# GlobalArrays/ga

Measured on AMD Instinct MI355X. Metric: GiB/s device-resident 2-D strided f64 accumulate, 64 MiB patch; % HBM peak, higher is better.
Workload: dtype f64; 1 GPU; H; patch=2-D f64 2048x4096 patch, ld 8192 (64 MiB payload), payload_bytes=67108864, parallelism=owner-aligned x1 (no collective)

## Files before the change

### ga_amd/_lib.py

```python
import ctypes
import os

_HERE = os.path.dirname(os.path.abspath(__file__))
LIB_PATH = os.path.join(_HERE, "libga_amd.so")
GA_LIB_PATH = os.path.join(_HERE, "libga_amd_ga.so")
DIAG_LIB_PATH = os.path.join(_HERE, "libga_amd_diag.so")

c_int_p = ctypes.POINTER(ctypes.c_int)
c_ll_p = ctypes.POINTER(ctypes.c_longlong)


class DoubleComplex(ctypes.Structure):
    _fields_ = [("real", ctypes.c_double), ("imag", ctypes.c_double)]


class SingleComplex(ctypes.Structure):
    _fields_ = [("real", ctypes.c_float), ("imag", ctypes.c_float)]


c_void_pp = ctypes.POINTER(ctypes.c_void_p)

SIGNATURES = {
    "comex_init": (ctypes.c_int, []),
    "comex_init_args": (ctypes.c_int, [c_int_p, ctypes.c_void_p]),
# ... 333 lines not shown
    "gaamd_iov_path_counts": (ctypes.c_int, [ctypes.POINTER(ctypes.c_ulonglong)]),
    "gaamd_host_parallel": (ctypes.c_int, [ctypes.c_int, ctypes.CFUNCTYPE(None, ctypes.c_int, ctypes.c_void_p),
                                           ctypes.c_void_p]),
    "gaamd_one_pass_count": (ctypes.c_ulonglong, []),
    "gaamd_segment_cache_reuse": (ctypes.c_ulonglong, []),
    "gaamd_segment_remaps": (ctypes.c_ulonglong, []),
    "gaamd_segment_cache_trims": (ctypes.c_ulonglong, []),
    "gaamd_segment_kind": (ctypes.c_int, [ctypes.c_void_p]),
    "gaamd_vmm_access_retries": (ctypes.c_ulonglong, []),
    "gaamd_vmm_exchange_selftest": (ctypes.c_int, [ctypes.c_int]),
    "gaamd_owner_counts": (ctypes.c_int, [ctypes.POINTER(ctypes.c_ulonglong)]),
    "gaamd_peers_unmapped": (ctypes.c_int, []),
    "gaamd_plan_strided": (ctypes.c_int, [ctypes.c_int, ctypes.c_void_p, c_int_p, ctypes.c_void_p, c_int_p, c_int_p,
                                          ctypes.c_int, ctypes.c_ulonglong, ctypes.c_ulonglong,
                                          ctypes.POINTER(ctypes.c_longlong)]),
    "gaamd_set_tuning": (ctypes.c_int, [ctypes.c_char_p, ctypes.c_int]),
    "gaamd_get_tuning": (ctypes.c_int, [ctypes.c_char_p]),
    "gaamd_device_count": (ctypes.c_int, []),
    "gaamd_set_device": (ctypes.c_int, [ctypes.c_int]),
    "gaamd_stream": (ctypes.c_void_p, []),
    "gaamd_stream_at": (ctypes.c_void_p, [ctypes.c_int]),
    "gaamd_dev_malloc": (ctypes.c_void_p, [ctypes.c_size_t]),
    "gaamd_dev_free": (ctypes.c_int, [ctypes.c_void_p]),
    "gaamd_host_malloc": (ctypes.c_void_p, [ctypes.c_size_t]),
    "gaamd_host_free": (ctypes.c_int, [ctypes.c_void_p]),
    "gaamd_memcpy": (ctypes.c_int, [ctypes.c_void_p, ctypes.c_void_p, ctypes.c_size_t]),
    "gaamd_memcpy2d": (ctypes.c_int, [ctypes.c_void_p, ctypes.c_size_t, ctypes.c_void_p, ctypes.c_size_t,
                                      ctypes.c_size_t, ctypes.c_size_t]),
    "gaamd_memset": (ctypes.c_int, [ctypes.c_void_p, ctypes.c_int, ctypes.c_size_t]),
    "gaamd_sync": (ctypes.c_int, [ctypes.c_void_p]),
# ... 178 lines not shown
```

### ga_amd/csrc/comex.cpp

```cpp
#include "comex_impl.hpp"
#include "../../include/ga_amd.h"
#include <hip/hip_version.h>
#include <stdio.h>
#include <stdlib.h>
#include <string.h>
#include <time.h>
#include <unistd.h>
#include <sched.h>
#include <deque>
#include <memory>
#include <algorithm>

#ifndef GAAMD_ROCM_PATH
#define GAAMD_ROCM_PATH "/opt/rocm"
#endif

namespace gaamd {

static std::vector<std::vector<int>> g_groups;

std::vector<int> group_members(int group) {
    Runtime &r = rt();
    std::vector<int> m;
    if (group == COMEX_GROUP_WORLD) {
// ... 345 lines not shown
            dv.dev = remote_view(world, dst, dlo, dhi);
            dv.hbm = segment_kind_of(world, (const char *)dst + dlo) == 1;
        } else {
            sv.dev = remote_view(world, src, slo, shi);
            sv.hbm = segment_kind_of(world, (const char *)src + slo) == 1;
            dv = local_view(dst, dlo, dhi, true, true);
        }
    } else {
        local_views(src, slo, shi, dst, dlo, dhi, sv, dv, hdl != nullptr);
    }
    if (dv.bounce) view_rows(dv, ds, count, levels, kind == X_ACC ? rb : count[0]);
    const bool bounce_only = (needs_sync(sv) || needs_sync(dv)) && !sv.staged && !dv.staged;
    const bool host_side = (needs_sync(sv) || needs_sync(dv)) && !bounce_only;
    const bool peer = kind == X_GET && world != r.rank && r.peer_src(world);
    if (peer) g_peer_gets.fetch_add(1, std::memory_order_relaxed);
    int si = 0;
    hipStream_t st;
    {
        std::lock_guard<std::mutex> g(r.launch_mu);
        stamp(1);
        if (host_side) sched_join_write(span_of(dv.dev, dlo, dhi));
        else si = sched_pick(span_of(sv.dev, slo, shi), span_of(dv.dev, dlo, dhi), payload_bytes(rb, count, levels));
        st = r.streams[si];
        stamp(2);
        int rc = launch_strided(cop, scale, sv.dev, ss, dv.dev, ds, count, levels, st, last_launch_info(), 0, ~0ull,
                                false, peer);
        stamp(3);
        if (rc == kErrPeerOrdered) rc = get_via_scratch(sv.dev, ss, dv.dev, ds, count, levels, st);
        if (rc) fatal("strided %s launch failed (code %d): misaligned elements or bad descriptor",
                      kind == X_ACC ? "acc" : (kind == X_PUT ? "put" : "get"), rc);
        if (host_side) sched_sync_all();
    }
    const bool synced = host_side || bounce_only || (!hdl && r.blocking_sync);
    if (!host_side && synced) {
        if (dv.hbm) sched_wait_flag(si);
        else GA_HIP(hipStreamSynchronize(st));
    }
    if (world != r.rank && !synced && !r.direct_pending.empty()) r.direct_pending[world] = 1;
    if (r.debug)
        fprintf(stderr, "[ga_amd %d] %s -> %d levels %d count0 %d rows %d: src %s dst %s stream %d\n", r.rank,
                kind == X_ACC ? "acc" : (kind == X_PUT ? "put" : "get"), world, levels, count[0],
// ... 620 lines not shown
        return 0;
    }
    if (!strcmp(key, "vmm_window")) {
        if (!out || nout < 2) return -1;
        vmm_window_usage(&out[0], &out[1]);
        return 0;
    }
    if (!strcmp(key, "pinned_threads")) {
        if (out && nout >= 1) out[0] = views_pinned_threads();
        return 0;
    }
    if (!strcmp(key, "iov_host_sides")) {
        if (out && nout >= 1) out[0] = g_iov_host_sides.load(std::memory_order_relaxed);
        return 0;
    }
    return -1;
}

int gaamd_iov_path_counts(unsigned long long counts[4]) {
    for (int k = 0; k < 4; ++k) counts[k] = g_iov_path[k].load(std::memory_order_relaxed);
    return 0;
}

int gaamd_toggle_counts(unsigned long long counts[3]) {
    for (int k = 0; k < 3; ++k) counts[k] = g_toggle[k].load(std::memory_order_relaxed);
    return 0;
}

int gaamd_route_counts(unsigned long long counts[4]) {
    for (int k = 0; k < 4; ++k) counts[k] = g_route[k].load(std::memory_order_relaxed);
// ... 9 lines not shown
```

### ga_amd/csrc/gaamd_kernels.h

```cpp
#pragma once
#include <stdint.h>
#include <hip/hip_runtime.h>
#include "../../include/comex.h"

namespace gaamd {

constexpr int kMaxLevels = 7;
constexpr int kOpCopy = 0;

struct FastDiv {
    uint32_t d, m, s;
    __host__ __device__ inline uint32_t div(uint32_t n) const {
#if defined(__HIP_DEVICE_COMPILE__)
        uint32_t hi = __umulhi(n, m);
#else
        uint32_t hi = (uint32_t)(((uint64_t)n * m) >> 32);
#endif
        return (uint32_t)(((uint64_t)hi + n) >> s);
    }
};
FastDiv make_fastdiv(uint32_t d);

struct alignas(16) Scale16 { uint64_t w[2]; };

// ... 30 lines not shown
Tuning &tuning();

struct LaunchInfo {
    int kind;
    int width;
    int unroll;
    int launches;
    uint64_t blocks;
    int block;
    int levels;
    int aligned;
    int sys;
};

constexpr int kErrPeerOrdered = -10;
int launch_strided(int op, const void *scale, const void *src, const int *src_stride,
                   void *dst, const int *dst_stride, const int *count, int stride_levels,
                   hipStream_t stream, LaunchInfo *info,
                   uint64_t row_begin = 0, uint64_t row_end = ~0ull, bool plan_only = false,
                   bool src_peer = false);

void side_span_host(const int *stride, const int *count, int stride_levels, int64_t row_bytes,
                    int64_t *lo, int64_t *hi);

int elem_size(int op);

constexpr int kPatchMaxLevels = 6;
constexpr int kPatchErrNdim = -2;
constexpr int kPatchErrCount = -3;
constexpr int kPatchErrOp = -4;
constexpr int kPatchErrScalar = -5;
constexpr int kPatchErrStride = -6;
constexpr int kPatchErrRange = -7;
constexpr int kPatchErrAlign = -8;
constexpr int kPatchErrOverlap = -11;
// ... 159 lines not shown
```

### ga_amd/csrc/gaamd_kernels.hip

```cpp
#pragma clang fp contract(off)

#include "gaamd_kernels.h"
#include "gaamd_device.hpp"
#include <string.h>
#include <algorithm>
#include <type_traits>
#include <atomic>
#include <vector>
#include <utility>
#include <mutex>
#include <cmath>

namespace gaamd {

FastDiv make_fastdiv(uint32_t d) {
    FastDiv f;
    f.d = d ? d : 1;
    uint32_t l = 0;
    while ((1ull << l) < f.d) ++l;
    f.s = l;
    f.m = (uint32_t)((((1ull << 32) * ((1ull << l) - f.d)) / f.d) + 1);
    return f;
}

// ... 105 lines not shown
        const int64_t c0 = (int64_t)chunk * (BS * U) - shift;
        const bool full = c0 >= 0 && c0 + BS * U <= (int64_t)d.nvec;
        chunk_op<OP, W, U, BS, SYS>(sp, dp, c0 + threadIdx.x, d.nvec, full, op);
    }
}

struct Desc2D {
    const char *src;
    char *dst;
    int64_t s_str, d_str;
    FastDiv chunk_div;
    uint32_t row0;
};

template <class OP, int W, int BS, bool SYS = false>
__global__ __launch_bounds__(BS) void k_rows2d(const Desc2D d, const OP op) {
    const uint32_t w = blockIdx.x;
    const uint32_t rl = d.chunk_div.div(w);
    const uint32_t chunk = w - rl * d.chunk_div.d;
    const int64_t r = (int64_t)(d.row0 + rl);
    const int64_t v = (int64_t)chunk * BS + threadIdx.x;
    const char *sp = d.src + r * d.s_str + v * W;
    char *dp = d.dst + r * d.d_str + v * W;
    typename Vec<W>::T a, b;
    if constexpr (SYS) {
        if constexpr (OP::kReadsDst) b = vload<W, true>(dp);
        a = vload_sys<W>(sp);
        if constexpr (!OP::kReadsDst) b = a;
    } else {
        a = vload<W, true>(sp);
        b = a;
        if constexpr (OP::kReadsDst) b = vload<W, true>(dp);
    }
    vstore<W, kNtStore>(dp, op.template apply<W>(b, a));
}

template <int LV>
struct DescND {
    const char *src;
    char *dst;
    int64_t s_str[LV], d_str[LV];
    FastDiv cnt[LV];
    FastDiv chunk_div;
    uint32_t row0;
};

template <class OP, int W, int BS, int LV>
__global__ __launch_bounds__(BS) void k_rowsnd(const DescND<LV> d, const OP op) {
    const uint32_t w = blockIdx.x;
// ... 366 lines not shown
static int flat_block_threads(int W) { return W == 16 ? 64 : 256; }
static uint64_t flat_block_items(int W) { return W == 16 ? 64 : 256ull * 4; }

template <int W> struct DefaultU { static constexpr int value = W == 16 ? 1 : (W == 8 ? 2 : (W == 4 ? 4 : 8)); };
static int unroll_for(int W) {
    switch (W) {
    case 16: return DefaultU<16>::value;
    case 8: return DefaultU<8>::value;
    case 4: return DefaultU<4>::value;
    case 2: return DefaultU<2>::value;
    default: return DefaultU<1>::value;
    }
}
constexpr int kSysBS = 256;

template <class OP, int W, int BS, bool SYS = false>
static hipError_t go_rows2(const Desc &d, const OP &op, uint64_t blocks, hipStream_t st) {
    constexpr int U = DefaultU<W>::value;
    Desc2 e;
    e.src = d.src;
    e.dst = d.dst;
    e.s_str = d.levels ? d.s_str[0] : 0;
    e.d_str = d.levels ? d.d_str[0] : 0;
    e.row0 = d.row0;
    e.nvec = d.nvec;
    e.chunks = d.chunks;
    e.items = (uint32_t)d.items;
    e.chunk_div = d.chunk_div;
    e.align_mask = d.align_mask;
    if constexpr (U == 1) {
        if (!d.align_mask && blocks == e.items && d.nvec % (uint32_t)BS == 0) {
            Desc2D f;
            f.src = d.src;
            f.dst = d.dst;
            f.s_str = e.s_str;
            f.d_str = e.d_str;
            f.chunk_div = d.chunk_div;
            f.row0 = d.row0;
            hipLaunchKernelGGL((k_rows2d<OP, W, BS, SYS>), dim3((uint32_t)blocks), dim3(BS), 0, st, f, op);
            return hipGetLastError();
        }
    }
    hipLaunchKernelGGL((k_rows2<OP, W, U, BS, SYS>), dim3((uint32_t)blocks), dim3(BS), 0, st, e, op);
    return hipGetLastError();
}

// ... 117 lines not shown
}

static hipError_t dispatch(int op, const void *scale, const Plan &p, const Desc &d, uint64_t blocks, hipStream_t st) {
    switch (op) {
    case kOpCopy: return dispatch_op(p, d, CopyOp{}, blocks, st);
    case COMEX_ACC_INT: { AccInt o; int32_t s; memcpy(&s, scale, 4); o.s = (uint32_t)s; return dispatch_op(p, d, o, blocks, st); }
    case COMEX_ACC_LNG: { AccLng o; int64_t s; memcpy(&s, scale, 8); o.s = (uint64_t)s; return dispatch_op(p, d, o, blocks, st); }
    case COMEX_ACC_FLT: { AccFlt o; memcpy(&o.s, scale, 4); return dispatch_op(p, d, o, blocks, st); }
    case COMEX_ACC_DBL: { AccDbl o; memcpy(&o.s, scale, 8); return dispatch_op(p, d, o, blocks, st); }
    case COMEX_ACC_CPL: { AccCpl o; float s[2]; memcpy(s, scale, 8); o.sr = s[0]; o.si = s[1]; return dispatch_op(p, d, o, blocks, st); }
    case COMEX_ACC_DCP: { AccDcp o; double s[2]; memcpy(s, scale, 16); o.sr = s[0]; o.si = s[1]; return dispatch_op(p, d, o, blocks, st); }
    }
    return hipErrorInvalidValue;
}


static bool rows_may_overlap(const int64_t *str, const uint32_t *cnt, int L, int64_t row_bytes) {
    int64_t s[kMaxLevels];
    uint32_t c[kMaxLevels];
    int n = 0;
    for (int j = 0; j < L; ++j)
        if (cnt[j] > 1) { s[n] = str[j] < 0 ? -str[j] : str[j]; c[n] = cnt[j]; ++n; }
    for (int i = 1; i < n; ++i)
        for (int k = i; k > 0 && s[k] < s[k - 1]; --k) { std::swap(s[k], s[k - 1]); std::swap(c[k], c[k - 1]); }
    int64_t extent = row_bytes;
    for (int i = 0; i < n; ++i) {
        if (s[i] < extent) return true;
        extent = s[i] * (int64_t)(c[i] - 1) + extent;
    }
    return false;
// ... 167 lines not shown

void side_span_host(const int *stride, const int *count, int stride_levels, int64_t row_bytes,
                    int64_t *lo, int64_t *hi) {
    int64_t str[kMaxLevels];
    uint32_t cnt[kMaxLevels];
    for (int j = 0; j < stride_levels && j < kMaxLevels; ++j) {
        str[j] = stride[j];
        cnt[j] = count[j + 1] < 0 ? 0 : (uint32_t)count[j + 1];
    }
    side_span(str, cnt, stride_levels, row_bytes, *lo, *hi);
}

int launch_strided(int op, const void *scale, const void *src, const int *src_stride,
                   void *dst, const int *dst_stride, const int *count, int stride_levels,
                   hipStream_t stream, LaunchInfo *info, uint64_t row_begin, uint64_t row_end, bool plan_only,
                   bool src_peer) {
    const Tuning &tn = g_tuning;
    if (info) memset(info, 0, sizeof(*info));
    if (stride_levels < 0 || stride_levels > kMaxLevels) return -2;
    if (!count || count[0] <= 0) return -3;
    const int esz = elem_size(op);
    if (!esz) return -4;
    if (op != kOpCopy && !scale) return -5;
    if (stride_levels > 0 && (!src_stride || !dst_stride)) return -6;

    int64_t row_bytes = (op == kOpCopy) ? count[0] : (int64_t)(count[0] / esz) * esz;
    uint64_t rows = 1;
    for (int j = 1; j <= stride_levels; ++j) {
        if (count[j] < 0) return -3;
        rows *= (uint64_t)count[j];
    }
// ... 119 lines not shown
        for (int j = 0; j < L; ++j) any = any || (ds[j] & (int64_t)d.align_mask) != 0;
        if (!any) d.align_mask = 0;
    }
    d.chunks = (d.nvec + per_chunk - 1 + (d.align_mask ? per_chunk - 1 : 0)) / per_chunk;
    d.chunk_div = make_fastdiv(d.chunks);

    const uint64_t lim = (1ull << 31) - 1;
    uint64_t rows_per_launch = rows;
    if (kind == KK_ROWS) rows_per_launch = std::min<uint64_t>(rows, lim / d.chunks);
    if (kind == KK_FLAT) rows_per_launch = std::min<uint64_t>(rows, lim / d.nvec);
    if (kind == KK_SERIAL || kind == KK_ORDERED) rows_per_launch = rows;
    if (rows_per_launch == 0) return -9;

    int launches = 0;
    uint64_t total_blocks = 0;
    for (uint64_t r0 = row_begin; r0 < row_end; r0 += rows_per_launch) {
        const uint64_t nr = std::min<uint64_t>(rows_per_launch, row_end - r0);
        d.row0 = (uint32_t)r0;
        d.rows = (uint32_t)nr;
        uint64_t blocks = 1;
        if (kind == KK_ROWS) {
            d.items = nr * d.chunks;
            blocks = d.items;
            if (src_peer && L > 1 && blocks > 65536) blocks = 65536;
        } else if (kind == KK_FLAT) {
            d.items = nr * d.nvec;
            const uint64_t per = flat_block_items(W);
            blocks = (d.items + per - 1) / per;
        } else {
            d.items = nr;
            if (p.variant == 4) {
                const uint32_t gx = (d.nvec + 255u) / 256u;
                blocks = (uint64_t)gx * cols_sum_slices(gx, (uint32_t)nr);
            }
            else if (p.variant == 3)
                blocks = (uint64_t)((d.nvec + 255u) / 256u) * ((nr + kColsAtomicRows - 1) / kColsAtomicRows);
            else if (p.cw) blocks = (d.nvec + (uint32_t)p.cw - 1) / (uint32_t)p.cw;
            else if (p.variant) blocks = (d.nvec + 63u) / 64u;
        }
        if (blocks > lim) blocks = lim;
        if (!plan_only) {
            hipError_t e = dispatch(op, scale, p, d, blocks, stream);
            if (e != hipSuccess) return -100 - (int)e;
        }
        ++launches;
        total_blocks += blocks;
    }
    if (!plan_only) g_kind_count[kind] += (unsigned long long)launches;
    if (info) {
        info->kind = kind;
        info->width = W;
        info->unroll = (kind == KK_ROWS) ? U : (kind == KK_ORDERED ? p.variant : 0);
        info->launches = launches;
        info->blocks = total_blocks;
        info->block = (kind == KK_ROWS) ? BS
                      : (kind == KK_FLAT ? flat_block_threads(W)
                                         : ((kind == KK_ORDERED && !p.variant) ? kOrderedBS
                                            : (p.variant == 4 || p.variant == 3 ? 256 : (p.cw ? KC_NW * 64 : 64))));
        info->levels = L;
        info->aligned = d.align_mask ? 1 : 0;
        info->sys = src_peer ? 1 : 0;
    }
    return 0;
}

}
```

### ga_amd/csrc/plumbing.hip

```cpp
#include "gaamd_kernels.h"
#include "runtime.hpp"
#include <string.h>
#include <stdlib.h>
#include <dlfcn.h>

namespace gaamd {

LaunchInfo g_last;
LaunchInfo *last_launch_info() { return &g_last; }

static hipStream_t stream_of(void *s) {
    if (s) return (hipStream_t)s;
    Runtime &r = rt();
    if (r.stream) return r.stream;
    return nullptr;
}

__device__ __forceinline__ uint64_t splitmix64_at(uint64_t seed, uint64_t i) {
    uint64_t z = seed + (i + 1) * 0x9E3779B97F4A7C15ULL;
    z = (z ^ (z >> 30)) * 0xBF58476D1CE4E5B9ULL;
    z = (z ^ (z >> 27)) * 0x94D049BB133111EBULL;
    return z ^ (z >> 31);
}

__global__ __launch_bounds__(256) void k_fill(void *dst, long n, int type, uint64_t seed) {
    for (long i = (long)blockIdx.x * blockDim.x + threadIdx.x; i < n; i += (long)gridDim.x * blockDim.x) {
// ... 302 lines not shown
    if (!strcmp(key, "flat_line_min")) return &t.flat_line_min;
    if (!strcmp(key, "ordered_cols")) return &t.ordered_cols;
    if (!strcmp(key, "iov_lds")) return &t.iov_lds;
    return nullptr;
}

int gaamd_set_tuning(const char *key, int value) {
    if (!strcmp(key, "streams")) {
        Runtime &r = rt();
        if (!r.initialized || value < 1 || value > 8) return -1;
        std::lock_guard<std::mutex> g(r.launch_mu);
        const int old = (int)r.streams.size();
        sched_resize(value);
        return old;
    }
    int *f = tuning_field(key);
    if (!f) return -1;
    if (!strcmp(key, "block") && value != 0 && value != 64 && value != 128) return -1;
    const int old = *f;
    *f = value;
    return old;
}

int gaamd_get_tuning(const char *key) {
    if (!strcmp(key, "streams")) return (int)rt().streams.size();
    int *f = tuning_field(key);
    return f ? *f : -1;
}

int gaamd_device_count(void) {
    int n = 0;
    if (hipGetDeviceCount(&n) != hipSuccess) {
        (void)hipGetLastError();
        return 0;
    }
    return n;
}

int gaamd_set_device(int dev) { return hipSetDevice(dev) == hipSuccess ? 0 : -1; }
void *gaamd_stream(void) { return rt().stream; }
// ... 16 lines not shown
    hipDeviceptr_t base = nullptr;
    size_t size = 0;
    if (hipMemGetAddressRange(&base, &size, (hipDeviceptr_t)p) == hipSuccess) addr_event('f', p, size, -1);
    else (void)hipGetLastError();
    return hipFree(p) == hipSuccess ? 0 : -1;
}

void *gaamd_host_malloc(size_t bytes) {
    void *p = nullptr;
    if (hipHostMalloc(&p, bytes, hipHostMallocMapped | hipHostMallocPortable) != hipSuccess) return nullptr;
    return p;
}
int gaamd_host_free(void *p) { return hipHostFree(p) == hipSuccess ? 0 : -1; }

int gaamd_memcpy(void *dst, const void *src, size_t bytes) {
    return hipMemcpy(dst, src, bytes, hipMemcpyDefault) == hipSuccess ? 0 : -1;
}
int gaamd_memcpy2d(void *dst, size_t dpitch, const void *src, size_t spitch, size_t width, size_t height) {
    return hipMemcpy2D(dst, dpitch, src, spitch, width, height, hipMemcpyDefault) == hipSuccess ? 0 : -1;
}
int gaamd_memset(void *dst, int value, size_t bytes) {
    return hipMemset(dst, value, bytes) == hipSuccess ? 0 : -1;
}
int gaamd_sync(void *stream) {
    Runtime &r = rt();
    if (!stream && r.initialized) {
        std::lock_guard<std::mutex> g(r.launch_mu);
        sched_sync_all();
        return 0;
    }
    hipStream_t s = stream_of(stream);
    hipError_t e = s ? hipStreamSynchronize(s) : hipDeviceSynchronize();
    return e == hipSuccess ? 0 : -(int)e;
}

int gaamd_join(void) {
// ... 63 lines not shown
```

### ga_amd/csrc/runtime.hpp

```cpp
#pragma once
#include <stdint.h>
#include <stddef.h>
#include <atomic>
#include <vector>
#include <mutex>
#include <thread>
#include <hip/hip_runtime_api.h>
#include "../../include/ga_amd.h"

namespace gaamd {

[[noreturn]] void fatal(const char *fmt, ...);
void trace(int level, const char *fmt, ...) __attribute__((format(printf, 2, 3)));

#define GA_HIP(call)                                                                  \
    do {                                                                              \
        hipError_t e_ = (call);                                                       \
        if (e_ != hipSuccess)                                                         \
            ::gaamd::fatal("%s failed: %s (%s:%d)", #call, hipGetErrorString(e_),     \
                           __FILE__, __LINE__);                                       \
    } while (0)

#define GA_ASSERT(cond, msg)                                                          \
    do {                                                                              \
// ... 145 lines not shown

Runtime &rt();

void boot_init();
void boot_allgather(const void *send, void *recv, size_t bytes);
void boot_barrier();
void boot_finalize();

void segment_cache_flush();
void sched_init(int nstreams, int pull_streams = 0);
void sched_fini();
void sched_resize(int nstreams);
void own_write_guard(const Span &dst);
int sched_pick(const Span &src, const Span &dst, uint64_t payload = 0, int prefer = -1);
void sched_join();
void sched_wait_flag(int s);
void sched_flag_init();
void sched_flag_fini();
void sched_join_write(const Span &dst);
void sched_sync_all();
void sched_publish_all();
extern std::atomic<bool> g_publish_conservative;
uint64_t sched_track(int s);
bool sched_complete(int s, uint64_t seq, bool wait);
uint64_t sched_epoch();

void wire_init();
void wire_finalize();
void wire_detach();
bool wire_active();
// ... 29 lines not shown
```

### ga_amd/csrc/sched.cpp

```cpp
#include <atomic>
#include "runtime.hpp"
#include "gaamd_kernels.h"
#include <string.h>
#include <stdlib.h>
#include <deque>
#include <algorithm>

namespace gaamd {

namespace {
constexpr int kHist = 64;
struct Entry {
    int stream;
    Span src, dst;
};
std::vector<Entry> g_hist;
std::vector<hipEvent_t> g_ev;
int g_rr = 0;
int g_base = -1;
unsigned g_base_waited = 0;

inline bool overlap(const Span &a, const Span &b) { return a.lo < b.hi && b.lo < a.hi && a.lo < a.hi && b.lo < b.hi; }

constexpr uint64_t kMarkEvery = 16;
struct Mark {
    uint64_t seq;
    hipEvent_t ev;
};
struct Marks {
    uint64_t issued = 0, done = 0, marked = 0;
    std::deque<Mark> q;
};
std::vector<Marks> g_marks;
std::vector<hipEvent_t> g_mark_pool;
std::mutex g_marks_mu;

void marks_reset_done() {
    for (Marks &m : g_marks) {
        m.done = m.marked = m.issued;
        for (const Mark &k : m.q) g_mark_pool.push_back(k.ev);
        m.q.clear();
    }
}

void mark_now(int s) {
    Marks &m = g_marks[s];
    if (m.marked == m.issued) return;
    hipEvent_t e;
    if (g_mark_pool.empty()) GA_HIP(hipEventCreateWithFlags(&e, hipEventDisableTiming));
    else { e = g_mark_pool.back(); g_mark_pool.pop_back(); }
    GA_HIP(hipEventRecord(e, rt().streams[s]));
    m.q.push_back({m.issued, e});
    m.marked = m.issued;
}
}

uint64_t sched_track(int s) {
    std::lock_guard<std::mutex> g(g_marks_mu);
    if (s < 0 || s >= (int)g_marks.size()) return 0;
    Marks &m = g_marks[s];
    const uint64_t seq = ++m.issued;
    if (seq - m.marked >= kMarkEvery) mark_now(s);
    return seq;
}

bool sched_complete(int s, uint64_t seq, bool wait) {
    std::unique_lock<std::mutex> g(g_marks_mu);
    if (seq == 0 || s < 0 || s >= (int)g_marks.size()) return true;
    Marks &m = g_marks[s];
    if (seq <= m.done) return true;
    if (m.marked < seq) mark_now(s);
    while (!m.q.empty()) {
        const Mark k = m.q.front();
        hipError_t e = hipEventQuery(k.ev);
        if (e == hipErrorNotReady && wait) {
            g.unlock();
            e = hipEventSynchronize(k.ev);
            g.lock();
            if (m.q.empty() || m.q.front().ev != k.ev) {
                if (m.done >= seq) return true;
                continue;
// ... 22 lines not shown
    r.user_streams = n;
    n += pull;
    r.streams.assign(1, r.stream);
    for (int i = 1; i < n; ++i) {
        hipStream_t s;
        GA_HIP(hipStreamCreateWithFlags(&s, hipStreamDefault));
        r.streams.push_back(s);
    }
    g_ev.assign(n, nullptr);
    for (int i = 0; i < n; ++i) GA_HIP(hipEventCreateWithFlags(&g_ev[i], hipEventDisableTiming));
    std::lock_guard<std::mutex> g(g_marks_mu);
    g_marks.assign(n, Marks());
    g_hist.clear();
    g_rr = 0;
    g_base = -1;
    sched_flag_init();
}

void sched_resize(int n) {
    Runtime &r = rt();
    const int pull = (int)r.streams.size() - r.user_streams;
    sched_sync_all();
    sched_fini();
    r.streams.clear();
    sched_init(n, pull);
}

static std::vector<hipEvent_t> g_pub_ev;
std::atomic<bool> g_publish_conservative{false};

void sched_fini() {
    Runtime &r = rt();
    for (hipEvent_t e : g_pub_ev) (void)hipEventDestroy(e);
    g_pub_ev.clear();
    for (size_t i = 1; i < r.streams.size(); ++i) (void)hipStreamDestroy(r.streams[i]);
    for (hipEvent_t e : g_ev) (void)hipEventDestroy(e);
    g_ev.clear();
    std::lock_guard<std::mutex> g(g_marks_mu);
    marks_reset_done();
    for (hipEvent_t e : g_mark_pool) (void)hipEventDestroy(e);
    g_mark_pool.clear();
    g_marks.clear();
    r.streams.clear();
    g_hist.clear();
}

static void wait_on(int waiter, int producer) {
    Runtime &r = rt();
    GA_HIP(hipEventRecord(g_ev[producer], r.streams[producer]));
    GA_HIP(hipStreamWaitEvent(r.streams[waiter], g_ev[producer], 0));
}

void sched_join() {
    Runtime &r = rt();
    const int n = (int)r.streams.size();
    if (n > 1) {
        for (int x = 1; x < n; ++x) wait_on(0, x);
        for (int x = 1; x < n; ++x) wait_on(x, 0);
    }
    g_hist.clear();
    g_base = -1;
}

void sched_join_write(const Span &dst) {
    own_write_guard(dst);
    sched_join();
}

void sched_sync_all() {
    Runtime &r = rt();
    for (hipStream_t s : r.streams) GA_HIP(hipStreamSynchronize(s));
    for (uint8_t &p : r.direct_pending) p = 0;
    {
        std::lock_guard<std::mutex> g(g_marks_mu);
        marks_reset_done();
    }
    g_hist.clear();
    g_base = -1;
}

void sched_publish_all() {
    Runtime &r = rt();
    while (g_pub_ev.size() < r.streams.size()) {
        hipEvent_t e;
        GA_HIP(hipEventCreateWithFlags(&e, hipEventDisableTiming | hipEventReleaseToSystem));
        g_pub_ev.push_back(e);
    }
    for (size_t i = 0; i < r.streams.size(); ++i) GA_HIP(hipEventRecord(g_pub_ev[i], r.streams[i]));
    sched_sync_all();
}

namespace {
uint64_t *g_flag_host = nullptr, *g_flag_dev = nullptr;
std::vector<uint64_t> g_flag_seq;
}

void sched_flag_init() {
// ... 1 lines not shown
    GA_HIP(hipHostMalloc((void **)&g_flag_host, 64 * sizeof(uint64_t), hipHostMallocMapped | hipHostMallocCoherent));
    GA_HIP(hipHostGetDevicePointer((void **)&g_flag_dev, g_flag_host, 0));
    memset(g_flag_host, 0, 64 * sizeof(uint64_t));
    g_flag_seq.assign(64, 0);
    const int rc = launch_flag(g_flag_dev + 63, 0, rt().stream);
    if (rc) fatal("completion flag launch failed (%d)", rc);
    GA_HIP(hipStreamSynchronize(rt().stream));
}

void sched_wait_flag(int s) {
    Runtime &r = rt();
    uint64_t v;
    volatile uint64_t *f;
    {
        std::lock_guard<std::mutex> g(r.launch_mu);
        sched_flag_init();
        if (s < 0 || s >= 64) fatal("stream index %d out of range", s);
        v = ++g_flag_seq[s];
        const int rc = launch_flag(g_flag_dev + s, v, r.streams[s]);
        if (rc) fatal("completion flag launch failed (%d)", rc);
        f = g_flag_host + s;
    }
    for (unsigned long spins = 0; __atomic_load_n(f, __ATOMIC_ACQUIRE) < v; ++spins) {
        if ((spins & 0xfffff) == 0xfffff) {
            const hipError_t e = hipStreamQuery(r.streams[s]);
            if (e == hipSuccess) break;
            if (e != hipErrorNotReady) fatal("stream failed: %s", hipGetErrorString(e));
        }
        __builtin_ia32_pause();
    }
}

void sched_flag_fini() {
    if (g_flag_host) (void)hipHostFree(g_flag_host);
    g_flag_host = g_flag_dev = nullptr;
    g_flag_seq.clear();
}

constexpr uint64_t kBigPayload = 192ull << 20;
constexpr uint64_t kSmallPayload = 8ull << 20;

int sched_pick(const Span &src, const Span &dst, uint64_t payload, int prefer) {
    Runtime &r = rt();
    own_write_guard(dst);
    const int n = (int)r.streams.size();
    if (n <= 1) return 0;
    const int nu = std::max(1, std::min(r.user_streams, n));
    if ((int)g_hist.size() >= kHist) {
        const int s0 = g_hist.front().stream;
        bool one = g_base < 0 || g_base == s0;
        for (const Entry &e : g_hist) one = one && e.stream == s0;
        if (one) {
            g_hist.clear();
            if (g_base != s0) g_base_waited = 1u << s0;
            g_base = s0;
        } else {
            sched_join();
        }
// ... 16 lines not shown
        }
    } else {
        s = last;
        for (int x = 0; x < n; ++x)
            if (x != s && (mask & (1u << x))) wait_on(s, x);
    }
    if (g_base >= 0 && !(g_base_waited & (1u << s))) {
        wait_on(s, g_base);
        g_base_waited |= 1u << s;
        if (g_base_waited == (1u << n) - 1) g_base = -1;
    }
    g_hist.push_back({s, src, dst});
    return s;
}

}
```

### include/ga_amd.h

```cpp
#ifndef GA_AMD_H
#define GA_AMD_H

#include <stddef.h>

#if defined(__cplusplus)
extern "C" {
#endif

#define GAAMD_OP_COPY 0

typedef int (*gaamd_allgather_fn)(const void *send, void *recv, size_t bytes, void *ctx);
typedef int (*gaamd_barrier_fn)(void *ctx);
int gaamd_set_bootstrap(int rank, int size, int local_rank,
                        gaamd_allgather_fn allgather, gaamd_barrier_fn barrier, void *ctx);
#ifdef MPI_VERSION
int gaamd_set_bootstrap_comm(MPI_Comm comm);
#endif
int gaamd_bootstrap_selftest(int rounds);
int gaamd_rank(void);
int gaamd_size(void);
int gaamd_device(void);
int gaamd_device_topology(int *ranks_on_gpu, int *gpus_on_node, int *peer_loads);
int gaamd_node_info(int *node, int *nnodes, int *node_size);
int gaamd_wire_selftest(int rounds);
// ... 102 lines not shown
                    const void *src, long long lds, void *dst, long long ldd, void *stream);
int gaamd_transpose_acc(int op, long long m, long long n, const void *alpha,
                        const void *b, long long ldb, void *c, long long ldc, void *stream);
int gaamd_transpose_plan(int op, long long rows, long long cols, const void *src,
                         long long lds, const void *dst, long long ldd, long long plan[4]);
long gaamd_packed_size(const int *count, int stride_levels);
int gaamd_pack(const void *src, const int *src_stride, const int *count, int stride_levels,
               void *packed, void *stream);
int gaamd_unpack(const void *packed, void *dst, const int *dst_stride, const int *count,
                 int stride_levels, void *stream);
int gaamd_unpack_acc(int op, const void *scale, const void *packed, void *dst,
                     const int *dst_stride, const int *count, int stride_levels, void *stream);
int gaamd_plan_strided(int op, const void *src, const int *src_stride, const void *dst, const int *dst_stride,
                       const int *count, int stride_levels, unsigned long long row_begin,
                       unsigned long long row_end, long long plan[8]);
int gaamd_last_launch(int *kind, int *width, int *unroll, int *launches,
                      unsigned long long *blocks);
int gaamd_kernel_counts(unsigned long long counts[5]);
int gaamd_route_counts(unsigned long long counts[4]);
int gaamd_toggle_counts(unsigned long long counts[3]);
int gaamd_iov_path_counts(unsigned long long counts[4]);
int gaamd_host_parallel(int T, void (*fn)(int t, void *ctx), void *ctx);
unsigned long long gaamd_one_pass_count(void);
unsigned long long gaamd_segment_cache_reuse(void);
unsigned long long gaamd_segment_remaps(void);
unsigned long long gaamd_segment_cache_trims(void);
int gaamd_segment_kind(const void *p);
unsigned long long gaamd_vmm_access_retries(void);
int gaamd_vmm_exchange_selftest(int rounds);
int gaamd_peers_unmapped(void);
// ... 39 lines not shown
```

Before: 6070 GiB/s.

## Coalesce nonblocking local accumulates into batched multi-slot row kernels

Result: slower. 5837 GiB/s (-3.8%).

```diff
diff --git a/ga_amd/_lib.py b/ga_amd/_lib.py
--- a/ga_amd/_lib.py
+++ b/ga_amd/_lib.py
@@ -371,6 +371,7 @@
     "gaamd_plan_strided": (ctypes.c_int, [ctypes.c_int, ctypes.c_void_p, c_int_p, ctypes.c_void_p, c_int_p, c_int_p,
                                           ctypes.c_int, ctypes.c_ulonglong, ctypes.c_ulonglong,
                                           ctypes.POINTER(ctypes.c_longlong)]),
+    "gaamd_plan_coalesce": (ctypes.c_int, [ctypes.c_int, ctypes.c_int, c_ll_p, c_int_p, c_int_p]),
     "gaamd_set_tuning": (ctypes.c_int, [ctypes.c_char_p, ctypes.c_int]),
     "gaamd_get_tuning": (ctypes.c_int, [ctypes.c_char_p]),
     "gaamd_device_count": (ctypes.c_int, []),
diff --git a/ga_amd/csrc/comex.cpp b/ga_amd/csrc/comex.cpp
--- a/ga_amd/csrc/comex.cpp
+++ b/ga_amd/csrc/comex.cpp
@@ -383,17 +383,37 @@
     const bool host_side = (needs_sync(sv) || needs_sync(dv)) && !bounce_only;
     const bool peer = kind == X_GET && world != r.rank && r.peer_src(world);
     if (peer) g_peer_gets.fetch_add(1, std::memory_order_relaxed);
+    const bool coalescible = kind == X_ACC && hdl && world == r.rank && sched_coalesce_mode() != 0 && !r.one_pass &&
+                             sv.hbm && dv.hbm && !host_side && !bounce_only && !sv.ring && !sv.registered &&
+                             !sv.staged && !sv.bounce && !dv.registered && !dv.staged && !dv.bounce;
     int si = 0;
-    hipStream_t st;
+    hipStream_t st = nullptr;
     {
         std::lock_guard<std::mutex> g(r.launch_mu);
         stamp(1);
-        if (host_side) sched_join_write(span_of(dv.dev, dlo, dhi));
-        else si = sched_pick(span_of(sv.dev, slo, shi), span_of(dv.dev, dlo, dhi), payload_bytes(rb, count, levels));
-        st = r.streams[si];
-        stamp(2);
-        int rc = launch_strided(cop, scale, sv.dev, ss, dv.dev, ds, count, levels, st, last_launch_info(), 0, ~0ull,
+        int rc = 0;
+        bool planned = false;
+        if (coalescible) {
+            RowsOp ro;
+            rc = launch_strided(cop, scale, sv.dev, ss, dv.dev, ds, count, levels, nullptr, last_launch_info(), 0, ~0ull,
+                                false, false, &ro);
+            planned = rc == kDeferred;
+            if (planned) {
+                stamp(2);
+                si = sched_coalesce(span_of(sv.dev, slo, shi), span_of(dv.dev, dlo, dhi),
+                                    payload_bytes(rb, count, levels), ro);
+                st = r.streams[si];
+                rc = 0;
+            }
+        }
+        if (!planned) {
+            if (host_side) sched_join_write(span_of(dv.dev, dlo, dhi));
+            else si = sched_pick(span_of(sv.dev, slo, shi), span_of(dv.dev, dlo, dhi), payload_bytes(rb, count, levels));
+            st = r.streams[si];
+            stamp(2);
+            rc = launch_strided(cop, scale, sv.dev, ss, dv.dev, ds, count, levels, st, last_launch_info(), 0, ~0ull,
                                 false, peer);
+        }
         stamp(3);
         if (rc == kErrPeerOrdered) rc = get_via_scratch(sv.dev, ss, dv.dev, ds, count, levels, st);
         if (rc) fatal("strided %s launch failed (code %d): misaligned elements or bad descriptor",
@@ -1044,6 +1064,11 @@
         if (out && nout >= 1) out[0] = g_iov_host_sides.load(std::memory_order_relaxed);
         return 0;
     }
+    if (!strcmp(key, "coalesce")) {
+        if (!out || nout < 3) return -1;
+        sched_coalesce_counts(out);
+        return 0;
+    }
     return -1;
 }
 
diff --git a/ga_amd/csrc/gaamd_kernels.h b/ga_amd/csrc/gaamd_kernels.h
--- a/ga_amd/csrc/gaamd_kernels.h
+++ b/ga_amd/csrc/gaamd_kernels.h
@@ -68,11 +68,24 @@
 };
 
 constexpr int kErrPeerOrdered = -10;
+struct RowsOp {
+    const char *src;
+    char *dst;
+    int64_t s_str, d_str;
+    FastDiv chunk_div;
+    uint32_t row0;
+    uint32_t blocks;
+    int op, W, BS;
+    Scale16 scale;
+};
+constexpr int kRowsMultiMax = 8;
+constexpr int kDeferred = 1;
 int launch_strided(int op, const void *scale, const void *src, const int *src_stride,
                    void *dst, const int *dst_stride, const int *count, int stride_levels,
                    hipStream_t stream, LaunchInfo *info,
                    uint64_t row_begin = 0, uint64_t row_end = ~0ull, bool plan_only = false,
-                   bool src_peer = false);
+                   bool src_peer = false, RowsOp *defer = nullptr);
+int launch_rows_multi(const RowsOp *ops, int n, hipStream_t stream);
 
 void side_span_host(const int *stride, const int *count, int stride_levels, int64_t row_bytes,
                     int64_t *lo, int64_t *hi);
diff --git a/ga_amd/csrc/gaamd_kernels.hip b/ga_amd/csrc/gaamd_kernels.hip
--- a/ga_amd/csrc/gaamd_kernels.hip
+++ b/ga_amd/csrc/gaamd_kernels.hip
@@ -143,8 +143,7 @@
 };
 
 template <class OP, int W, int BS, bool SYS = false>
-__global__ __launch_bounds__(BS) void k_rows2d(const Desc2D d, const OP op) {
-    const uint32_t w = blockIdx.x;
+__device__ __forceinline__ void rows2d_body(const Desc2D &d, const OP &op, uint32_t w) {
     const uint32_t rl = d.chunk_div.div(w);
     const uint32_t chunk = w - rl * d.chunk_div.d;
     const int64_t r = (int64_t)(d.row0 + rl);
@@ -162,6 +161,34 @@
         if constexpr (OP::kReadsDst) b = vload<W, true>(dp);
     }
     vstore<W, kNtStore>(dp, op.template apply<W>(b, a));
+}
+
+template <class OP, int W, int BS, bool SYS = false>
+__global__ __launch_bounds__(BS) void k_rows2d(const Desc2D d, const OP op) {
+    rows2d_body<OP, W, BS, SYS>(d, op, blockIdx.x);
+}
+
+template <class OP>
+struct MultiSlot {
+    Desc2D d;
+    uint32_t blocks;
+    OP op;
+};
+template <class OP, int K>
+struct MultiArgs {
+    MultiSlot<OP> s[K];
+};
+
+template <class OP, int W, int BS, int K>
+__global__ __launch_bounds__(BS) void k_rows2d_multi(const MultiArgs<OP, K> m) {
+    static_assert(sizeof(MultiSlot<OP>) % 4 == 0, "slot of whole dwords");
+    const MultiSlot<OP> s = m.s[blockIdx.y];
+    uint32_t f[sizeof(MultiSlot<OP>) / 4];
+    __builtin_memcpy(f, &s, sizeof(s));
+#pragma unroll
+    for (unsigned i = 0; i < sizeof(MultiSlot<OP>) / 4; ++i) asm volatile("" ::"s"(f[i]));
+    if (blockIdx.x >= s.blocks) return;
+    rows2d_body<OP, W, BS, false>(s.d, s.op, blockIdx.x);
 }
 
 template <int LV>
@@ -558,6 +585,10 @@
 }
 constexpr int kSysBS = 256;
 
+static inline bool rows2d_applies(int U, const Desc &d, uint64_t blocks, int BS) {
+    return U == 1 && !d.align_mask && blocks == (uint32_t)d.items && d.nvec % (uint32_t)BS == 0;
+}
+
 template <class OP, int W, int BS, bool SYS = false>
 static hipError_t go_rows2(const Desc &d, const OP &op, uint64_t blocks, hipStream_t st) {
     constexpr int U = DefaultU<W>::value;
@@ -573,7 +604,7 @@
     e.chunk_div = d.chunk_div;
     e.align_mask = d.align_mask;
     if constexpr (U == 1) {
-        if (!d.align_mask && blocks == e.items && d.nvec % (uint32_t)BS == 0) {
+        if (rows2d_applies(U, d, blocks, BS)) {
             Desc2D f;
             f.src = d.src;
             f.dst = d.dst;
@@ -721,6 +752,66 @@
     return hipErrorInvalidValue;
 }
 
+static Desc2D desc2d_of(const RowsOp &o) {
+    Desc2D f;
+    f.src = o.src;
+    f.dst = o.dst;
+    f.s_str = o.s_str;
+    f.d_str = o.d_str;
+    f.chunk_div = o.chunk_div;
+    f.row0 = o.row0;
+    return f;
+}
+
+template <class OP, int BS, int K>
+static hipError_t go_rows_multi(const RowsOp *ops, int n, hipStream_t st) {
+    static_assert(sizeof(OP) <= sizeof(Scale16), "OP value fits the stored scale");
+    MultiArgs<OP, K> m;
+    memset(&m, 0, sizeof(m));
+    uint32_t gx = 0;
+    for (int k = 0; k < n; ++k) {
+        m.s[k].d = desc2d_of(ops[k]);
+        m.s[k].blocks = ops[k].blocks;
+        memcpy(&m.s[k].op, &ops[k].scale, sizeof(OP));
+        gx = std::max(gx, ops[k].blocks);
+    }
+    hipLaunchKernelGGL((k_rows2d_multi<OP, 16, BS, K>), dim3(gx, (uint32_t)n), dim3(BS), 0, st, m);
+    return hipGetLastError();
+}
+
+template <class OP>
+static hipError_t rows_multi_op(const RowsOp *ops, int n, hipStream_t st) {
+    const int BS = ops[0].BS;
+    if (n == 1) {
+        OP o;
+        memcpy(&o, &ops[0].scale, sizeof(OP));
+        const Desc2D f = desc2d_of(ops[0]);
+        if (BS == 64) hipLaunchKernelGGL((k_rows2d<OP, 16, 64, false>), dim3(ops[0].blocks), dim3(64), 0, st, f, o);
+        else hipLaunchKernelGGL((k_rows2d<OP, 16, 128, false>), dim3(ops[0].blocks), dim3(128), 0, st, f, o);
+        return hipGetLastError();
+    }
+    if (n <= 4) return BS == 64 ? go_rows_multi<OP, 64, 4>(ops, n, st) : go_rows_multi<OP, 128, 4>(ops, n, st);
+    return BS == 64 ? go_rows_multi<OP, 64, 8>(ops, n, st) : go_rows_multi<OP, 128, 8>(ops, n, st);
+}
+
+int launch_rows_multi(const RowsOp *ops, int n, hipStream_t stream) {
+    if (!ops || n < 1 || n > kRowsMultiMax) return -2;
+    for (int k = 0; k < n; ++k)
+        if (ops[k].op != ops[0].op || ops[k].W != 16 || ops[k].BS != ops[0].BS || (ops[k].BS != 64 && ops[k].BS != 128) ||
+            !ops[k].blocks)
+            return -3;
+    hipError_t e = hipErrorInvalidValue;
+    switch (ops[0].op) {
+    case COMEX_ACC_INT: e = rows_multi_op<AccInt>(ops, n, stream); break;
+    case COMEX_ACC_LNG: e = rows_multi_op<AccLng>(ops, n, stream); break;
+    case COMEX_ACC_FLT: e = rows_multi_op<AccFlt>(ops, n, stream); break;
+    case COMEX_ACC_DBL: e = rows_multi_op<AccDbl>(ops, n, stream); break;
+    case COMEX_ACC_CPL: e = rows_multi_op<AccCpl>(ops, n, stream); break;
+    case COMEX_ACC_DCP: e = rows_multi_op<AccDcp>(ops, n, stream); break;
+    default: return -4;
+    }
+    return e == hipSuccess ? 0 : -100 - (int)e;
+}
 
 static bool rows_may_overlap(const int64_t *str, const uint32_t *cnt, int L, int64_t row_bytes) {
     int64_t s[kMaxLevels];
@@ -918,7 +1009,7 @@
 int launch_strided(int op, const void *scale, const void *src, const int *src_stride,
                    void *dst, const int *dst_stride, const int *count, int stride_levels,
                    hipStream_t stream, LaunchInfo *info, uint64_t row_begin, uint64_t row_end, bool plan_only,
-                   bool src_peer) {
+                   bool src_peer, RowsOp *defer) {
     const Tuning &tn = g_tuning;
     if (info) memset(info, 0, sizeof(*info));
     if (stride_levels < 0 || stride_levels > kMaxLevels) return -2;
@@ -1068,6 +1159,7 @@
 
     int launches = 0;
     uint64_t total_blocks = 0;
+    bool deferred = false;
     for (uint64_t r0 = row_begin; r0 < row_end; r0 += rows_per_launch) {
         const uint64_t nr = std::min<uint64_t>(rows_per_launch, row_end - r0);
         d.row0 = (uint32_t)r0;
@@ -1093,14 +1185,29 @@
             else if (p.variant) blocks = (d.nvec + 63u) / 64u;
         }
         if (blocks > lim) blocks = lim;
-        if (!plan_only) {
+        if (defer && op != kOpCopy && kind == KK_ROWS && !src_peer && L <= 1 && r0 == row_begin &&
+            nr == row_end - row_begin && rows2d_applies(U, d, blocks, BS)) {
+            defer->src = d.src;
+            defer->dst = d.dst;
+            defer->s_str = L ? d.s_str[0] : 0;
+            defer->d_str = L ? d.d_str[0] : 0;
+            defer->chunk_div = d.chunk_div;
+            defer->row0 = d.row0;
+            defer->blocks = (uint32_t)blocks;
+            defer->op = op;
+            defer->W = W;
+            defer->BS = BS;
+            memset(&defer->scale, 0, sizeof(defer->scale));
+            memcpy(&defer->scale, scale, (size_t)esz);
+            deferred = true;
+        } else if (!plan_only && !defer) {
             hipError_t e = dispatch(op, scale, p, d, blocks, stream);
             if (e != hipSuccess) return -100 - (int)e;
         }
         ++launches;
         total_blocks += blocks;
     }
-    if (!plan_only) g_kind_count[kind] += (unsigned long long)launches;
+    if (defer ? deferred : !plan_only) g_kind_count[kind] += (unsigned long long)launches;
     if (info) {
         info->kind = kind;
         info->width = W;
@@ -1115,7 +1222,7 @@
         info->aligned = d.align_mask ? 1 : 0;
         info->sys = src_peer ? 1 : 0;
     }
-    return 0;
-}
-
-}
+    return deferred ? kDeferred : 0;
+}
+
+}
diff --git a/ga_amd/csrc/plumbing.hip b/ga_amd/csrc/plumbing.hip
--- a/ga_amd/csrc/plumbing.hip
+++ b/ga_amd/csrc/plumbing.hip
@@ -10,6 +10,7 @@
 LaunchInfo *last_launch_info() { return &g_last; }
 
 static hipStream_t stream_of(void *s) {
+    sched_flush_unlocked();
     if (s) return (hipStream_t)s;
     Runtime &r = rt();
     if (r.stream) return r.stream;
@@ -342,6 +343,13 @@
         sched_resize(value);
         return old;
     }
+    if (!strcmp(key, "coalesce")) {
+        if (value < 0 || value > 2) return -1;
+        std::lock_guard<std::mutex> g(rt().launch_mu);
+        const int old = sched_coalesce_mode();
+        sched_set_coalesce(value);
+        return old;
+    }
     int *f = tuning_field(key);
     if (!f) return -1;
     if (!strcmp(key, "block") && value != 0 && value != 64 && value != 128) return -1;
@@ -352,6 +360,7 @@
 
 int gaamd_get_tuning(const char *key) {
     if (!strcmp(key, "streams")) return (int)rt().streams.size();
+    if (!strcmp(key, "coalesce")) return sched_coalesce_mode();
     int *f = tuning_field(key);
     return f ? *f : -1;
 }
@@ -398,12 +407,15 @@
 int gaamd_host_free(void *p) { return hipHostFree(p) == hipSuccess ? 0 : -1; }
 
 int gaamd_memcpy(void *dst, const void *src, size_t bytes) {
+    sched_flush_unlocked();
     return hipMemcpy(dst, src, bytes, hipMemcpyDefault) == hipSuccess ? 0 : -1;
 }
 int gaamd_memcpy2d(void *dst, size_t dpitch, const void *src, size_t spitch, size_t width, size_t height) {
+    sched_flush_unlocked();
     return hipMemcpy2D(dst, dpitch, src, spitch, width, height, hipMemcpyDefault) == hipSuccess ? 0 : -1;
 }
 int gaamd_memset(void *dst, int value, size_t bytes) {
+    sched_flush_unlocked();
     return hipMemset(dst, value, bytes) == hipSuccess ? 0 : -1;
 }
 int gaamd_sync(void *stream) {
diff --git a/ga_amd/csrc/runtime.hpp b/ga_amd/csrc/runtime.hpp
--- a/ga_amd/csrc/runtime.hpp
+++ b/ga_amd/csrc/runtime.hpp
@@ -183,6 +183,13 @@
 void own_write_guard(const Span &dst);
 int sched_pick(const Span &src, const Span &dst, uint64_t payload = 0, int prefer = -1);
 void sched_join();
+struct RowsOp;
+int sched_coalesce_mode();
+void sched_set_coalesce(int mode);
+int sched_coalesce(const Span &src, const Span &dst, uint64_t payload, const RowsOp &op);
+void sched_flush();
+void sched_flush_unlocked();
+void sched_coalesce_counts(unsigned long long out[3]);
 void sched_wait_flag(int s);
 void sched_flag_init();
 void sched_flag_fini();
diff --git a/ga_amd/csrc/sched.cpp b/ga_amd/csrc/sched.cpp
--- a/ga_amd/csrc/sched.cpp
+++ b/ga_amd/csrc/sched.cpp
@@ -34,6 +34,9 @@
 std::vector<Marks> g_marks;
 std::vector<hipEvent_t> g_mark_pool;
 std::mutex g_marks_mu;
+
+std::atomic<int> g_held{0};
+void co_reset();
 
 void marks_reset_done() {
     for (Marks &m : g_marks) {
@@ -60,11 +63,12 @@
     if (s < 0 || s >= (int)g_marks.size()) return 0;
     Marks &m = g_marks[s];
     const uint64_t seq = ++m.issued;
-    if (seq - m.marked >= kMarkEvery) mark_now(s);
+    if (seq - m.marked >= kMarkEvery && !g_held.load(std::memory_order_acquire)) mark_now(s);
     return seq;
 }
 
 bool sched_complete(int s, uint64_t seq, bool wait) {
+    sched_flush_unlocked();
     std::unique_lock<std::mutex> g(g_marks_mu);
     if (seq == 0 || s < 0 || s >= (int)g_marks.size()) return true;
     Marks &m = g_marks[s];
@@ -117,6 +121,7 @@
     g_hist.clear();
     g_rr = 0;
     g_base = -1;
+    co_reset();
     sched_flag_init();
 }
 
@@ -134,6 +139,7 @@
 
 void sched_fini() {
     Runtime &r = rt();
+    sched_flush();
     for (hipEvent_t e : g_pub_ev) (void)hipEventDestroy(e);
     g_pub_ev.clear();
     for (size_t i = 1; i < r.streams.size(); ++i) (void)hipStreamDestroy(r.streams[i]);
@@ -156,6 +162,7 @@
 
 void sched_join() {
     Runtime &r = rt();
+    sched_flush();
     const int n = (int)r.streams.size();
     if (n > 1) {
         for (int x = 1; x < n; ++x) wait_on(0, x);
@@ -172,6 +179,7 @@
 
 void sched_sync_all() {
     Runtime &r = rt();
+    sched_flush();
     for (hipStream_t s : r.streams) GA_HIP(hipStreamSynchronize(s));
     for (uint8_t &p : r.direct_pending) p = 0;
     {
@@ -184,6 +192,7 @@
 
 void sched_publish_all() {
     Runtime &r = rt();
+    sched_flush();
     while (g_pub_ev.size() < r.streams.size()) {
         hipEvent_t e;
         GA_HIP(hipEventCreateWithFlags(&e, hipEventDisableTiming | hipEventReleaseToSystem));
@@ -215,6 +224,7 @@
     volatile uint64_t *f;
     {
         std::lock_guard<std::mutex> g(r.launch_mu);
+        sched_flush();
         sched_flag_init();
         if (s < 0 || s >= 64) fatal("stream index %d out of range", s);
         v = ++g_flag_seq[s];
@@ -243,6 +253,7 @@
 
 int sched_pick(const Span &src, const Span &dst, uint64_t payload, int prefer) {
     Runtime &r = rt();
+    sched_flush();
     own_write_guard(dst);
     const int n = (int)r.streams.size();
     if (n <= 1) return 0;
@@ -289,4 +300,182 @@
     return s;
 }
 
-}
+namespace {
+constexpr int kCoK = kRowsMultiMax;
+constexpr uint64_t kCoPayloadCap = 512ull << 20;
+constexpr double kCoGuardUs = 15.0;
+constexpr double kCoBytesPerUs = 6.0e6;
+constexpr uint64_t kCoTraffic = 3;
+
+struct CoOp {
+    Span src, dst;
+    int op, W, BS;
+    uint64_t payload;
+};
+struct CoBatch {
+    int n = 0;
+    uint64_t payload = 0;
+    CoOp ops[kCoK];
+};
+struct CoDecision {
+    bool close_first;
+    bool hold;
+    bool launch_after;
+};
+
+inline double co_after_launch(double drain_us, double now_us, uint64_t payload) {
+    return std::max(drain_us, now_us) + (double)(kCoTraffic * payload) / kCoBytesPerUs;
+}
+
+CoDecision co_decide(int mode, const CoBatch &b, const CoOp &o, double now_us, double drain_us) {
+    CoDecision d = {false, true, false};
+    if (b.n > 0) {
+        d.close_first = o.op != b.ops[0].op || o.W != b.ops[0].W || o.BS != b.ops[0].BS ||
+                        b.payload + o.payload > kCoPayloadCap;
+        for (int k = 0; k < b.n && !d.close_first; ++k)
+            d.close_first = overlap(o.dst, b.ops[k].dst) || overlap(o.dst, b.ops[k].src) || overlap(o.src, b.ops[k].dst);
+    }
+    const int n0 = d.close_first ? 0 : b.n;
+    const uint64_t p0 = d.close_first ? 0 : b.payload;
+    if (d.close_first) drain_us = co_after_launch(drain_us, now_us, b.payload);
+    if (n0 == 0 && mode == 1 && drain_us <= now_us) {
+        d.hold = false;
+        return d;
+    }
+    d.launch_after = n0 + 1 >= kCoK || p0 + o.payload >= kCoPayloadCap || (mode == 1 && drain_us - now_us < kCoGuardUs);
+    return d;
+}
+
+int g_co_mode = 1;
+bool g_co_env_read = false;
+CoBatch g_co;
+RowsOp g_co_rows[kCoK];
+int g_co_stream = 0;
+double g_co_drain_us = 0;
+std::atomic<unsigned long long> g_co_held_ops{0}, g_co_launches{0}, g_co_largest{0};
+
+double co_now_us() {
+    return std::chrono::duration<double, std::micro>(std::chrono::steady_clock::now().time_since_epoch()).count();
+}
+
+void co_reset() {
+    g_co.n = 0;
+    g_co.payload = 0;
+    g_co_drain_us = 0;
+    g_held.store(0, std::memory_order_release);
+    if (!g_co_env_read) {
+        g_co_env_read = true;
+        const char *e = getenv("COMEX_AMD_COALESCE");
+        if (e && *e) {
+            const int v = atoi(e);
+            if (v < 0 || v > 2) fatal("COMEX_AMD_COALESCE=%s: 0 (off), 1 (default) or 2 (always hold)", e);
+            g_co_mode = v;
+        }
+    }
+}
+
+void co_launch(const RowsOp *rows, int n, uint64_t payload, int s) {
+    const int rc = launch_rows_multi(rows, n, rt().streams[s]);
+    if (rc) fatal("coalesced accumulate launch failed (code %d, %d operations)", rc, n);
+    g_co_drain_us = co_after_launch(g_co_drain_us, co_now_us(), payload);
+}
+}
+
+int sched_coalesce_mode() { return g_co_mode; }
+void sched_set_coalesce(int mode) {
+    sched_flush();
+    g_co_mode = mode;
+}
+
+void sched_flush() {
+    if (!g_co.n) return;
+    const int n = g_co.n;
+    g_co.n = 0;
+    co_launch(g_co_rows, n, g_co.payload, g_co_stream);
+    g_co.payload = 0;
+    g_held.store(0, std::memory_order_release);
+    g_co_launches.fetch_add(1, std::memory_order_relaxed);
+    if ((unsigned long long)n > g_co_largest.load(std::memory_order_relaxed)) g_co_largest.store(n, std::memory_order_relaxed);
+}
+
+void sched_flush_unlocked() {
+    if (!g_held.load(std::memory_order_acquire)) return;
+    std::lock_guard<std::mutex> g(rt().launch_mu);
+    sched_flush();
+}
+
+void sched_coalesce_counts(unsigned long long out[3]) {
+    out[0] = g_co_held_ops.load(std::memory_order_relaxed);
+    out[1] = g_co_launches.load(std::memory_order_relaxed);
+    out[2] = g_co_largest.load(std::memory_order_relaxed);
+}
+
+int sched_coalesce(const Span &src, const Span &dst, uint64_t payload, const RowsOp &op) {
+    Runtime &r = rt();
+    const CoOp o = {src, dst, op.op, op.W, op.BS, payload};
+    if ((int)g_hist.size() >= kHist) sched_flush();
+    const CoDecision d = co_decide(g_co_mode, g_co, o, co_now_us(), g_co_drain_us);
+    if (d.close_first) sched_flush();
+    int s;
+    if (g_co.n == 0) {
+        s = sched_pick(src, dst, d.hold ? kBigPayload : payload);
+        if (!d.hold) {
+            co_launch(&op, 1, payload, s);
+            return s;
+        }
+        g_co_stream = s;
+    } else {
+        s = g_co_stream;
+        const int n = (int)r.streams.size();
+        unsigned mask = 0;
+        for (const Entry &e : g_hist)
+            if (overlap(dst, e.dst) || overlap(dst, e.src) || overlap(src, e.dst)) mask |= 1u << e.stream;
+        for (int x = 0; x < n; ++x)
+            if (x != s && (mask & (1u << x))) wait_on(s, x);
+        if (n > 1) g_hist.push_back({s, src, dst});
+    }
+    g_co_rows[g_co.n] = op;
+    g_co.ops[g_co.n] = o;
+    ++g_co.n;
+    g_co.payload += payload;
+    g_held.store(g_co.n, std::memory_order_release);
+    g_co_held_ops.fetch_add(1, std::memory_order_relaxed);
+    if (d.launch_after) sched_flush();
+    return s;
+}
+
+}
+
+extern "C" int gaamd_plan_coalesce(int mode, int n, const long long *ops, int *batch, int *launched_by) {
+    using namespace gaamd;
+    if ((mode != 1 && mode != 2) || n < 0 || (n > 0 && (!ops || !batch || !launched_by))) return -1;
+    CoBatch b;
+    int first = 0, launches = 0;
+    double drain = 0;
+    auto launch = [&](int upto, int by, double now) {
+        for (int i = first; i < upto; ++i) {
+            batch[i] = launches;
+            launched_by[i] = by;
+        }
+        drain = co_after_launch(drain, now, b.payload);
+        ++launches;
+        first = upto;
+        b.n = 0;
+        b.payload = 0;
+    };
+    for (int i = 0; i < n; ++i) {
+        const long long *v = ops + 9 * (size_t)i;
+        const CoOp o = {{v[0], v[1]}, {v[2], v[3]}, (int)v[4], (int)v[5], (int)v[6], (uint64_t)v[7]};
+        const double now = (double)v[8];
+        const CoDecision d = co_decide(mode, b, o, now, drain);
+        if (d.close_first) launch(i, i, now);
+        b.ops[b.n++] = o;
+        b.payload += o.payload;
+        if (!d.hold || d.launch_after) launch(i + 1, i, now);
+    }
+    for (int i = first; i < n; ++i) {
+        batch[i] = launches;
+        launched_by[i] = n;
+    }
+    return launches + (first < n ? 1 : 0);
+}
diff --git a/include/ga_amd.h b/include/ga_amd.h
--- a/include/ga_amd.h
+++ b/include/ga_amd.h
@@ -140,6 +140,7 @@
 int gaamd_plan_strided(int op, const void *src, const int *src_stride, const void *dst, const int *dst_stride,
                        const int *count, int stride_levels, unsigned long long row_begin,
                        unsigned long long row_end, long long plan[8]);
+int gaamd_plan_coalesce(int mode, int n, const long long *ops, int *batch, int *launched_by);
 int gaamd_last_launch(int *kind, int *width, int *unroll, int *launches,
                       unsigned long long *blocks);
 int gaamd_kernel_counts(unsigned long long counts[5]);
```
